# pairlab/leibnizgym

Measured on AMD Instinct MI355X. Metric: env-steps/sec (whole node), trifinger_difficulty_4 @65536 envs, 1/2/4/8 GPUs, higher is better.
Workload: dtype f32

## Files before the change

### leibnizgym_amd/csrc/tf_roles.h

```cpp
#pragma once
#include <type_traits>

#include "tf_contact.h"

#define NT 256

enum { M_ACT_IN = 1, M_RESETS = 2, M_TORQUE = 4, M_SIM = 8, M_POST = 16, M_FINISH = 32, M_ACT_RAND = 64  };
#define M_FUSED_STEP (M_ACT_IN | M_RESETS | M_TORQUE | M_SIM | M_POST | M_FINISH)
#define M_FUSED_STEP_RAND (M_FUSED_STEP | M_ACT_RAND)
#define M_FUSED_RESET (M_RESETS | M_TORQUE | M_SIM | M_POST)

#define L_REC(f) (30 * (f))
#define R_A 0
#define R_DIR 6
#define R_RXD 15
#define R_U 24
#define R_DL 27
#define P_AW 0
#define P_BW 3
#define P_MINV 6
#define P_S1 12
#define P_C1 13
#define P_P2 14
#define P_P3 17
// ... 1754 lines not shown
                    const Yaw ym = {m.base_yaw_cos[fm], m.base_yaw_sin[fm], 0.0f, 0.0f, m.base_height};
                    const float ex[3] = {pm.k.c1, 0.0f, -pm.k.s1};
                    float ey[3], aw[3], bw[3];
                    {
                        float g[3], xg[3], ez[3], ab[3], bb[3];
#pragma unroll
                        for (int i = 0; i < 3; ++i) g[i] = FMA(-jx, ex[i], pm.k.p3[i] - pm.k.p2[i]);
                        cross3(ex, g, xg);
#pragma unroll
                        for (int i = 0; i < 3; ++i) { ey[i] = FMA(jy, g[i], -(jz * xg[i])) * inv_j; ez[i] = FMA(jz, g[i], jy * xg[i]) * inv_j; }
#pragma unroll
                        for (int i = 0; i < 3; ++i) {
                            ab[i] = FMA(sh.a[2], ez[i], FMA(sh.a[1], ey[i], FMA(sh.a[0], ex[i], pm.k.p2[i])));
                            bb[i] = FMA(sh.b[2], ez[i], FMA(sh.b[1], ey[i], FMA(sh.b[0], ex[i], pm.k.p2[i])));
                        }
                        base_to_world(ym, ab, aw);
                        base_to_world(ym, bb, bw);
                    }
                    {
                        const int o = o_;
                        const int fd = (fm + o >= 3) ? fm + o - 3 : fm + o;
                        float Pm[3], Pd[3], sp;
                        {
                            float Ad[3], Bd[3];
#pragma unroll
                            for (int j = 0; j < 3; ++j) { Ad[j] = LD(L_REC(fd) + P_AW + j); Bd[j] = LD(L_REC(fd) + P_BW + j); }
                            seg_seg_s(aw, bw, Ad, Bd, Pm, Pd, sp);
                        }
                        const float dv[3] = {Pd[0] - Pm[0], Pd[1] - Pm[1], Pd[2] - Pm[2]};
                        const float dist2 = dot3(dv, dv);
                        const float inv = f_rsqrt(f_max(dist2, 1e-12f));
                        const float dist = dist2 * inv;
                        const float n[3] = {dv[0] * inv, dv[1] * inv, dv[2] * inv};
                        float nm[3];
                        dir_world_to_base(ym, n, nm);
                        const float u1 = dot3(nm, ex), u2 = dot3(nm, ey);
                        const float rho = FMA(sp, sh.rho[1] - sh.rho[0], sh.rho[0]);
                        const float h1 = FMA(sp, sh.w1[1] - sh.w1[0], sh.w1[0]) - rho, h2 = FMA(sp, sh.w2[1] - sh.w2[0], sh.w2[0]) - rho;
                        const float o1 = FMA(sp, sh.o1[1] - sh.o1[0], sh.o1[0]), o2 = FMA(sp, sh.o2[1] - sh.o2[0], sh.o2[0]);
                        const float ext = FMA(o2, u2, FMA(o1, u1, FMA(h2, f_abs(u2), FMA(h1, f_abs(u1), rho))));
                        const float gap = dist - ext - m.cap_radius;
                        if ((dist2 > 1e-12f) && (gap < m.contact_margin)) {
                            float Jd[3], Wd[3], Jm[3], Wm[3], vd[3], vm[3];
                            {
                                const Yaw yd = {m.base_yaw_cos[fd], m.base_yaw_sin[fd], 0.0f, 0.0f, m.base_height};
                                FingerPubRegs pd;
                                read_pub(lds, lane, fd, pd);
                                float C[3], Cb_[3], L1[3], L2[3], L3[3], nb[3];
#pragma unroll
                                for (int j = 0; j < 3; ++j) C[j] = FMA(-m.cap_radius, n[j], Pd[j]);
                                world_to_base(yd, C, Cb_);
                                levers(pd.k, Cb_, L1, L2, L3);
                                dir_world_to_base(yd, n, nb);
                                Jd[0] = dot3(L1, nb); Jd[1] = dot3(L2, nb); Jd[2] = dot3(L3, nb);
                                sym3_mul(pd.k.Minv, Jd, Wd);
                            }
                            {
                                float C[3], Cb_[3], L1[3], L2[3], L3[3];
#pragma unroll
                                for (int j = 0; j < 3; ++j) C[j] = FMA(ext, n[j], Pm[j]);
                                world_to_base(ym, C, Cb_);
                                levers(pm.k, Cb_, L1, L2, L3);
                                Jm[0] = dot3(L1, nm); Jm[1] = dot3(L2, nm); Jm[2] = 0.0f;
                                sym3_mul(pm.k.Minv, Jm, Wm);
                            }
#pragma unroll
                            for (int j = 0; j < 3; ++j) { vd[j] = LD(L_REC(fd) + P_VQ + j); vm[j] = LD(L_REC(fm) + P_VQ + j); }
                            const float vn0 = dot3(Jd, vd) - dot3(Jm, vm);
                            if (contact_live(m, gap, vn0, h)) {
                                const float bias = contact_bias(m, gap, vn0, inv_h, rest_ff);
                                const float lam = f_max(-(vn0 + bias) * f_rcp2(dot3(Jd, Wd) + dot3(Jm, Wm)), 0.0f);
#pragma unroll
                                for (int j = 0; j < 3; ++j) {
                                    const float dd = Wd[j] * lam, dm = Wm[j] * lam;
                                    if (dd != 0.0f) LD(L_VQFF + 3 * fd + j) = LD(L_VQFF + 3 * fd + j) + dd;
                                    if (dm != 0.0f) LD(L_VQFF + 3 * fm + j) = LD(L_VQFF + 3 * fm + j) - dm;
                                }
                            }
                        }
                    }
                }
            }
            STAMP(sb_ + 2);
            BAR();
            STAMP(sb_ + 3);
            if constexpr (WIDE) {
#include "tf_floor_corners.inc"
            }
            STAMP(sb_ + 4);
            BAR();
            STAMP(sb_ + 5);
            if constexpr (WIDE && !BOXK) {
            Twist tw;
#pragma unroll
            for (int j = 0; j < 3; ++j) { tw.p[j].x = v[j]; tw.p[j].y = w[j]; }
            float2v mI; mI.x = inv_m; mI.y = inv_I;
            float cDinv[9], cbias[3], clam[9], Km[9];
            float2v rec[27];
#pragma unroll
            for (int f = 0; f < 3; ++f) {
                const int rb = L_REC(f);
                cbias[f] = LD(L_INIT + f);
#pragma unroll
                for (int d = 0; d < 3; ++d) { cDinv[3 * f + d] = LD(L_VQFF + 3 * f + d); clam[3 * f + d] = LD(rb + R_DL + d); Km[3 * f + d] = LD(rb + R_A + d); }
#pragma unroll
                for (int j = 0; j < 9; ++j) { rec[9 * f + j].x = LD(rb + R_DIR + j); rec[9 * f + j].y = LD(rb + R_RXD + j); }
                if (cDinv[3 * f] > 0.0f) {
#pragma unroll
                    for (int d = 0; d < 3; ++d) pk_row_apply_neg(&rec[9 * f + 3 * d], clam[3 * f + d], mI, tw);
                }
            }
#pragma unroll
            for (int c = 0; c < 4; ++c) {
                if (fDinv[3 * c] > 0.0f) {
                    cz_apply(&fr_[3 * c], flam[3 * c], mI, tw);
                    cx_apply(&fr_[3 * c], flam[3 * c + 1], mI, tw);
                    cy_apply(&fr_[3 * c], flam[3 * c + 2], mI, tw);
                }
            }
#pragma unroll
            for (int c = 0; c < 4; ++c) {
                const int wb = L_WALL + 12 * c;
                if (c < 2) {
                    if (slot_any[c] && w_D[3 * c] > 0.0f) {
                        wn_apply(&w_n[2 * c], &w_a[3 * c], w_lam[3 * c], mI, tw);
                        wt_apply(&w_n[2 * c], &w_b[3 * c], w_lam[3 * c + 1], mI, tw);
                        cz_apply(&w_r[3 * c], w_lam[3 * c + 2], mI, tw);
                    }
                } else if (slot_any[c] && LD(wb + 5) > 0.0f) {
                    float r[3] = {LD(wb), LD(wb + 1), LD(wb + 2)}, n[2] = {LD(wb + 3), LD(wb + 4)};
                    float a[3], b[3];
                    wall_arm_n(r, n, a);
                    wall_arm_t(r, n, b);
                    wn_apply(n, a, LD(wb + 9), mI, tw);
                    wt_apply(n, b, LD(wb + 10), mI, tw);
                    cz_apply(r, LD(wb + 11), mI, tw);
                }
            }
            if constexpr (SURF) {
                if (__builtin_expect(cone_any != 0u, 0)) {
#pragma unroll 1
                    for (int c = 0; c < 4; ++c) {
                        const int cb = L_CONE + 22 * c, wb = L_WALL + 12 * c;
                        if (((cone_any >> c) & 1u) && LD(cb + 18) > 0.0f) {
#pragma unroll 1
                            for (int d = 0; d < 3; ++d) pk_row_apply_lds(lds, lane, cb + 6 * d, LD(wb + 9 + d), mI, tw);
                        }
                    }
                }
            }
            uint32_t t_wait = 0u, t_fc = 0u, t_floor = 0u;
            STAMP(sb_ + 9);
            for (int it = 0; it < P.iters; ++it) {
                const uint32_t tf0_ = NOW();
                const bool last = it == P.iters - 1;
                float uu[9];
#pragma unroll
                for (int f = 0; f < 3; ++f) {
#pragma unroll
                    for (int j = 0; j < 3; ++j) uu[3 * f + j] = LD(L_REC(f) + R_U + j);
                }
#pragma unroll
                for (int f = 0; f < 3; ++f) {
#ifdef TF_DIAG_NO_FC
                    if (false) {
#else
                    if (cDinv[3 * f] > 0.0f) {
#endif
                        const int rb = L_REC(f);
                        const float2v* R = &rec[9 * f];
                        float vr[3], dl[3];
                        {
                            float2v p0 = R[0] * tw.p[0], p1 = R[3] * tw.p[0], p2 = R[6] * tw.p[0];
                            p0 = pk_fma(R[1], tw.p[1], p0); p1 = pk_fma(R[4], tw.p[1], p1); p2 = pk_fma(R[7], tw.p[1], p2);
                            p0 = pk_fma(R[2], tw.p[2], p0); p1 = pk_fma(R[5], tw.p[2], p1); p2 = pk_fma(R[8], tw.p[2], p2);
                            vr[0] = uu[3 * f] - (p0.x + p0.y); vr[1] = uu[3 * f + 1] - (p1.x + p1.y); vr[2] = uu[3 * f + 2] - (p2.x + p2.y);
                        }
                        dl[0] = solve_normal(clam[3 * f], cDinv[3 * f], vr[0], cbias[f]);
                        vr[1] = FMA(Km[3 * f], dl[0], vr[1]);
                        dl[1] = solve_tangent(clam[3 * f + 1], cDinv[3 * f + 1], vr[1], mu_fc * clam[3 * f]);
                        vr[2] = FMA(Km[3 * f + 2], dl[1], FMA(Km[3 * f + 1], dl[0], vr[2]));
                        dl[2] = solve_tangent(clam[3 * f + 2], cDinv[3 * f + 2], vr[2], mu_fc * clam[3 * f]);
#pragma unroll
                        for (int d = 0; d < 3; ++d) {
                            LD(rb + R_DL + d) = dl[d];
                            pk_row_apply_neg(&R[3 * d], dl[d], mI, tw);
                        }
                    }
                }
                t_fc += NOW() - tf0_;
                { const uint32_t t0_ = NOW(); BAR(); t_wait += NOW() - t0_; }
#pragma unroll
                for (int c = 0; c < 4; ++c) {
                    const float* r = &fr_[3 * c];
#ifdef TF_DIAG_NO_FLOOR
                    if (false) {
#else
                    if (fDinv[3 * c] > 0.0f) {
#endif
                        float dl = solve_normal(flam[3 * c], fDinv[3 * c], cz_vrel(r, tw), fbias[c]);
                        cz_apply(r, dl, mI, tw);
                        dl = solve_tangent(flam[3 * c + 1], fDinv[3 * c + 1], cx_vrel(r, tw), mu_cf * flam[3 * c]);
                        cx_apply(r, dl, mI, tw);
                        dl = solve_tangent(flam[3 * c + 2], fDinv[3 * c + 2], cy_vrel(r, tw), mu_cf * flam[3 * c]);
                        cy_apply(r, dl, mI, tw);
                    }
                }
                t_floor += NOW() - tf0_;
#pragma unroll
                for (int c = 0; c < 4; ++c) {
#ifdef TF_DIAG_NO_WALL
                    continue;
#endif
                    if (!slot_any[c]) continue;
                    const int wb = L_WALL + 12 * c;
                    if (c < 2) {
                        float dl = solve_normal(w_lam[3 * c], w_D[3 * c], wn_vrel(&w_n[2 * c], &w_a[3 * c], tw), w_bias[c]);
                        wn_apply(&w_n[2 * c], &w_a[3 * c], dl, mI, tw);
                        dl = solve_tangent(w_lam[3 * c + 1], w_D[3 * c + 1], wt_vrel(&w_n[2 * c], &w_b[3 * c], tw), mu_cw * w_lam[3 * c]);
                        wt_apply(&w_n[2 * c], &w_b[3 * c], dl, mI, tw);
                        dl = solve_tangent(w_lam[3 * c + 2], w_D[3 * c + 2], cz_vrel(&w_r[3 * c], tw), mu_cw * w_lam[3 * c]);
                        cz_apply(&w_r[3 * c], dl, mI, tw);
                        if (last && w_D[3 * c] > 0.0f) {
#pragma unroll
                            for (int d = 0; d < 3; ++d) LD(wb + 9 + d) = w_lam[3 * c + d];
                        }
                    } else {
                        float r[3] = {LD(wb), LD(wb + 1), LD(wb + 2)}, n[2] = {LD(wb + 3), LD(wb + 4)};
                        float Dinv[3] = {LD(wb + 5), LD(wb + 6), LD(wb + 7)}, bias = LD(wb + 8);
                        float lam[3] = {LD(wb + 9), LD(wb + 10), LD(wb + 11)};
                        float a[3], b[3];
                        wall_arm_n(r, n, a);
                        wall_arm_t(r, n, b);
                        float dl = solve_normal(lam[0], Dinv[0], wn_vrel(n, a, tw), bias);
                        wn_apply(n, a, dl, mI, tw);
                        dl = solve_tangent(lam[1], Dinv[1], wt_vrel(n, b, tw), mu_cw * lam[0]);
                        wt_apply(n, b, dl, mI, tw);
                        dl = solve_tangent(lam[2], Dinv[2], cz_vrel(r, tw), mu_cw * lam[0]);
                        cz_apply(r, dl, mI, tw);
                        if (Dinv[0] > 0.0f) {
#pragma unroll
                            for (int d = 0; d < 3; ++d) LD(wb + 9 + d) = lam[d];
                        }
                    }
                }
                if constexpr (SURF) {
                    if (__builtin_expect(cone_any != 0u, 0)) {
#pragma unroll
                    for (int c = 0; c < 4; ++c) {
                        const int cb = L_CONE + 22 * c, wb = L_WALL + 12 * c;
                        if (((cone_any >> c) & 1u) && LD(cb + 18) > 0.0f) {
                            float lim = 0.0f;
#pragma unroll
                            for (int d = 0; d < 3; ++d) {
                                const float vr = pk_row_vel_lds(lds, lane, cb + 6 * d, tw);
                                float lam = LD(wb + 9 + d);
                                const float dl = (d == 0) ? solve_normal(lam, LD(cb + 18), vr, LD(cb + 21)) : solve_tangent(lam, LD(cb + 18 + d), vr, lim);
                                lim = (d == 0) ? mu_cw * lam : lim;
                                LD(wb + 9 + d) = lam;
                                pk_row_apply_lds(lds, lane, cb + 6 * d, dl, mI, tw);
                            }
                        }
                    }
                    }
                }
                if (last) {
#pragma unroll
                    for (int f = 0; f < 3; ++f) {
                        const int rb = L_REC(f);
                        float ftv[3] = {0.0f, 0.0f, 0.0f}, Fc[3] = {0.0f, 0.0f, 0.0f};
                        if (cDinv[3 * f] > 0.0f) {
#pragma unroll
                            for (int j = 0; j < 3; ++j) {
                                ftv[j] = FMA(rec[9 * f + 6 + j].x, clam[3 * f + 2], rec[9 * f + 3 + j].x * clam[3 * f + 1]);
                                Fc[j] = FMA(rec[9 * f + j].x, clam[3 * f], ftv[j]) * inv_h;
                            }
                        }
                        LD(L_INIT + f) = clam[3 * f];
#pragma unroll
                        for (int j = 0; j < 3; ++j) { LD(rb + R_A + j) = ftv[j]; LD(rb + R_A + 3 + j) = Fc[j]; }
                    }
                }
                { const uint32_t t0_ = NOW(); BAR(); t_wait += NOW() - t0_; }
            }
            STAMP(sb_ + 6);
            STAMPV(sb_ + 8, t_wait);
            STAMPV(sb_ + 10, t_fc);
            STAMPV(sb_ + 11, t_floor);
#pragma unroll
            for (int j = 0; j < 3; ++j) { v[j] = tw.p[j].x; w[j] = tw.p[j].y; }
            } else {
            float cDinv[9], cbias[3], clam[9];
            constexpr int NRR = WIDE ? 27 : 1, NRA = WIDE ? 9 : 1;
            float rA[NRA], rDir[NRR], rRxd[NRR];
            if (WIDE) {
#pragma unroll
                for (int f = 0; f < 3; ++f) {
#pragma unroll
                    for (int j = 0; j < 3; ++j) rA[(3 * f + j) % NRA] = LD(L_REC(f) + R_A + j);
#pragma unroll
                    for (int j = 0; j < 9; ++j) { rDir[(9 * f + j) % NRR] = LD(L_REC(f) + R_DIR + j); rRxd[(9 * f + j) % NRR] = LD(L_REC(f) + R_RXD + j); }
                }
            }
#pragma unroll
            for (int f = 0; f < 3; ++f) {
                const int rb = L_REC(f);
                cbias[f] = LD(L_INIT + f);
#pragma unroll
                for (int d = 0; d < 3; ++d) { cDinv[3 * f + d] = LD(L_VQFF + 3 * f + d); clam[3 * f + d] = LD(rb + R_DL + d); }
                if (cDinv[3 * f] > 0.0f) {
#pragma unroll
                    for (int d = 0; d < 3; ++d) {
                        float dir[3], rxd[3];
#pragma unroll
                        for (int j = 0; j < 3; ++j) { dir[j] = WIDE ? rDir[(9 * f + 3 * d + j) % NRR] : LD(rb + R_DIR + 3 * d + j); rxd[j] = WIDE ? rRxd[(9 * f + 3 * d + j) % NRR] : LD(rb + R_RXD + 3 * d + j); }
                        float sc = clam[3 * f + d] * inv_m, qq = clam[3 * f + d] * inv_I;
#pragma unroll
                        for (int j = 0; j < 3; ++j) { v[j] = FMA(-dir[j], sc, v[j]); w[j] = FMA(-rxd[j], qq, w[j]); }
                    }
                }
            }
#pragma unroll
            for (int c = 0; c < 4; ++c) {
                if (fDinv[3 * c] > 0.0f) {
                    if (__builtin_expect(box, 0)) {
                        float S[6];
#pragma unroll
                        for (int e = 0; e < 6; ++e) S[e] = LD(L_POSE_S + e);
#pragma unroll
                        for (int d = 0; d < 3; ++d) {
                            float n[3], a[3];
                            box_axis(d, n);
                            box_arm(S, &fr_[3 * c], n, a);
                            g_apply(n, a, flam[3 * c + d], inv_m, inv_I, v, w);
                        }
                    } else {
                        cz_apply(&fr_[3 * c], flam[3 * c], inv_m, inv_I, v, w);
                        cx_apply(&fr_[3 * c], flam[3 * c + 1], inv_m, inv_I, v, w);
                        cy_apply(&fr_[3 * c], flam[3 * c + 2], inv_m, inv_I, v, w);
                    }
                }
            }
            {
#pragma unroll
            for (int c = 0; c < 4; ++c) {
                const int wb = L_WALL + 12 * c;
                if (WREG && c < 2) {
                    if (slot_any[c] && w_D[3 * c] > 0.0f) {
                        wn_apply(&w_n[2 * c], &w_a[3 * c], w_lam[3 * c], inv_m, inv_I, v, w);
                        wt_apply(&w_n[2 * c], &w_b[3 * c], w_lam[3 * c + 1], inv_m, inv_I, v, w);
                        cz_apply(&w_r[3 * c], w_lam[3 * c + 2], inv_m, inv_I, v, w);
                    }
                } else
                if (slot_any[c] && LD(wb + 5) > 0.0f) {
                    float r[3] = {LD(wb), LD(wb + 1), LD(wb + 2)}, n[2] = {LD(wb + 3), LD(wb + 4)};
                    float a[3], b[3], c3[3];
                    wall_arms(box, lds, lane, r, n, a, b, c3);
                    wn_apply(n, a, LD(wb + 9), inv_m, inv_I, v, w);
                    wt_apply(n, b, LD(wb + 10), inv_m, inv_I, v, w);
                    if (__builtin_expect(box, 0)) { float ez[3]; box_axis(0, ez); g_apply(ez, c3, LD(wb + 11), inv_m, inv_I, v, w); }
                    else cz_apply(r, LD(wb + 11), inv_m, inv_I, v, w);
                }
            }
            }
            uint32_t t_wait = 0u, t_fc = 0u, t_floor = 0u;
            STAMP(sb_ + 9);
            for (int it = 0; it < P.iters; ++it) {
                const uint32_t tf0_ = NOW();
                const bool last = it == P.iters - 1;
                float uu[9];
                if (WIDE) {
#pragma unroll
                    for (int f = 0; f < 3; ++f) {
#pragma unroll
                        for (int j = 0; j < 3; ++j) uu[3 * f + j] = LD(L_REC(f) + R_U + j);
                    }
                }
#pragma unroll
                for (int f = 0; f < 3; ++f) {
                    const int rb = L_REC(f);
                    if (cDinv[3 * f] > 0.0f) {
                        float Km[3], u[3], dirs[9], rxds[9], vr[3], dl[3];
#pragma unroll
                        for (int j = 0; j < 3; ++j) { Km[j] = WIDE ? rA[(3 * f + j) % NRA] : LD(rb + R_A + j); u[j] = WIDE ? uu[3 * f + j] : LD(rb + R_U + j); }
#pragma unroll
                        for (int j = 0; j < 9; ++j) { dirs[j] = WIDE ? rDir[(9 * f + j) % NRR] : LD(rb + R_DIR + j); rxds[j] = WIDE ? rRxd[(9 * f + j) % NRR] : LD(rb + R_RXD + j); }
#pragma unroll
                        for (int d = 0; d < 3; ++d) vr[d] = u[d] - (dot3(&dirs[3 * d], v) + dot3(&rxds[3 * d], w));
                        dl[0] = solve_normal(clam[3 * f], cDinv[3 * f], vr[0], cbias[f]);
                        vr[1] = FMA(Km[0], dl[0], vr[1]);
                        dl[1] = solve_tangent(clam[3 * f + 1], cDinv[3 * f + 1], vr[1], mu_fc * clam[3 * f]);
                        vr[2] = FMA(Km[2], dl[1], FMA(Km[1], dl[0], vr[2]));
                        dl[2] = solve_tangent(clam[3 * f + 2], cDinv[3 * f + 2], vr[2], mu_fc * clam[3 * f]);
#pragma unroll
                        for (int d = 0; d < 3; ++d) {
                            LD(rb + R_DL + d) = dl[d];
                            const float sc = dl[d] * inv_m, qq = dl[d] * inv_I;
#pragma unroll
                            for (int j = 0; j < 3; ++j) { v[j] = FMA(-dirs[3 * d + j], sc, v[j]); w[j] = FMA(-rxds[3 * d + j], qq, w[j]); }
                        }
                    }
                }
                t_fc += NOW() - tf0_;
                { const uint32_t t0_ = NOW(); BAR(); t_wait += NOW() - t0_; }
#pragma unroll
                for (int c = 0; c < 4; ++c) {
                    const float* r = &fr_[3 * c];
                    if (__builtin_expect(box, 0)) {
                        if (fDinv[3 * c] > 0.0f) {
                            float S[6];
#pragma unroll
                            for (int e = 0; e < 6; ++e) S[e] = LD(L_POSE_S + e);
#pragma unroll
                            for (int d = 0; d < 3; ++d) {
                                float n[3], a[3];
                                box_axis(d, n);
                                box_arm(S, r, n, a);
                                const float vrel = g_vrel(n, a, v, w);
                                const float dlb = (d == 0) ? solve_normal(flam[3 * c], fDinv[3 * c], vrel, fbias[c])
                                                           : solve_tangent(flam[3 * c + d], fDinv[3 * c + d], vrel, mu_cf * flam[3 * c]);
                                g_apply(n, a, dlb, inv_m, inv_I, v, w);
                            }
                        }
                    } else
                    if (fDinv[3 * c] > 0.0f) {
                        float dl = solve_normal(flam[3 * c], fDinv[3 * c], cz_vrel(r, v, w), fbias[c]);
                        cz_apply(r, dl, inv_m, inv_I, v, w);
                        dl = solve_tangent(flam[3 * c + 1], fDinv[3 * c + 1], cx_vrel(r, v, w), mu_cf * flam[3 * c]);
                        cx_apply(r, dl, inv_m, inv_I, v, w);
                        dl = solve_tangent(flam[3 * c + 2], fDinv[3 * c + 2], cy_vrel(r, v, w), mu_cf * flam[3 * c]);
                        cy_apply(r, dl, inv_m, inv_I, v, w);
                    }
                }
                t_floor += NOW() - tf0_;
                {
#pragma unroll
                for (int c = 0; c < 4; ++c) {
                    if (!slot_any[c]) continue;
                    const int wb = L_WALL + 12 * c;
                    if (WREG && c < 2) {
                        float dl = solve_normal(w_lam[3 * c], w_D[3 * c], wn_vrel(&w_n[2 * c], &w_a[3 * c], v, w), w_bias[c]);
                        wn_apply(&w_n[2 * c], &w_a[3 * c], dl, inv_m, inv_I, v, w);
                        dl = solve_tangent(w_lam[3 * c + 1], w_D[3 * c + 1], wt_vrel(&w_n[2 * c], &w_b[3 * c], v, w), mu_cw * w_lam[3 * c]);
                        wt_apply(&w_n[2 * c], &w_b[3 * c], dl, inv_m, inv_I, v, w);
                        dl = solve_tangent(w_lam[3 * c + 2], w_D[3 * c + 2], cz_vrel(&w_r[3 * c], v, w), mu_cw * w_lam[3 * c]);
                        cz_apply(&w_r[3 * c], dl, inv_m, inv_I, v, w);
                        if (last && w_D[3 * c] > 0.0f) {
#pragma unroll
                            for (int d = 0; d < 3; ++d) LD(wb + 9 + d) = w_lam[3 * c + d];
                        }
                    } else {
                        float r[3] = {LD(wb), LD(wb + 1), LD(wb + 2)}, n[2] = {LD(wb + 3), LD(wb + 4)};
                        float Dinv[3] = {LD(wb + 5), LD(wb + 6), LD(wb + 7)}, bias = LD(wb + 8);
                        float lam[3] = {LD(wb + 9), LD(wb + 10), LD(wb + 11)};
                        float a[3], b[3], c3[3];
                        wall_arms(box, lds, lane, r, n, a, b, c3);
                        float dl = solve_normal(lam[0], Dinv[0], wn_vrel(n, a, v, w), bias);
                        wn_apply(n, a, dl, inv_m, inv_I, v, w);
                        dl = solve_tangent(lam[1], Dinv[1], wt_vrel(n, b, v, w), mu_cw * lam[0]);
                        wt_apply(n, b, dl, inv_m, inv_I, v, w);
                        if (__builtin_expect(box, 0)) {
                            float ez[3];
                            box_axis(0, ez);
                            dl = solve_tangent(lam[2], Dinv[2], g_vrel(ez, c3, v, w), mu_cw * lam[0]);
                            g_apply(ez, c3, dl, inv_m, inv_I, v, w);
                        } else {
                            dl = solve_tangent(lam[2], Dinv[2], cz_vrel(r, v, w), mu_cw * lam[0]);
                            cz_apply(r, dl, inv_m, inv_I, v, w);
                        }
                        if (Dinv[0] > 0.0f) {
#pragma unroll
                            for (int d = 0; d < 3; ++d) LD(wb + 9 + d) = lam[d];
                        }
                    }
                }
                }
                if (last) {
#pragma unroll
                    for (int f = 0; f < 3; ++f) {
                        const int rb = L_REC(f);
                        float ftv[3] = {0.0f, 0.0f, 0.0f}, Fc[3] = {0.0f, 0.0f, 0.0f};
                        if (cDinv[3 * f] > 0.0f) {
                            float dirs[9];
#pragma unroll
                            for (int j = 0; j < 9; ++j) dirs[j] = WIDE ? rDir[(9 * f + j) % NRR] : LD(rb + R_DIR + j);
#pragma unroll
                            for (int j = 0; j < 3; ++j) {
                                ftv[j] = FMA(dirs[6 + j], clam[3 * f + 2], dirs[3 + j] * clam[3 * f + 1]);
                                Fc[j] = FMA(dirs[j], clam[3 * f], ftv[j]) * inv_h;
                            }
                        }
                        LD(L_INIT + f) = clam[3 * f];
#pragma unroll
                        for (int j = 0; j < 3; ++j) { LD(rb + R_A + j) = ftv[j]; LD(rb + R_A + 3 + j) = Fc[j]; }
                    }
                }
                { const uint32_t t0_ = NOW(); BAR(); t_wait += NOW() - t0_; }
            }
            STAMP(sb_ + 6);
            STAMPV(sb_ + 8, t_wait);
            STAMPV(sb_ + 10, t_fc);
            STAMPV(sb_ + 11, t_floor);
            }
#pragma unroll
            for (int j = 0; j < 12; ++j) lam_cf[j] = flam[j];
            if (__builtin_expect(box, 0)) {
                float S[6], ww[3];
#pragma unroll
                for (int e = 0; e < 6; ++e) S[e] = LD(L_POSE_S + e);
                sym3_mul(S, w, ww);
#pragma unroll
                for (int j = 0; j < 3; ++j) w[j] = ww[j];
            }
#pragma unroll
            for (int j = 0; j < 3; ++j) {
                cv[j] = v[j]; cw[j] = w[j];
                cp[j] = FMA(h, v[j], cp[j]);
            }
            quat_integrate(cq, cw, h);
            STAMP(sb_ + 7);
        }
#pragma unroll
        for (int c = 0; c < 4; ++c) {
#pragma unroll
            for (int d = 0; d < 3; ++d) lam_cw[3 * c + d] = LD(L_WALL + 12 * c + 9 + d);
        }
        __builtin_amdgcn_s_setprio(0);
    }
    STAMP(30);
    StatsTicket tk;
    tk.mine = 0ull; tk.old = 0ull;
    if (MODE & (M_POST | M_FINISH)) {
        c_reset = P.reset_buf[(unsigned)cx.i] != 0;
        c_goal_reset = P.goal_reset_buf[(unsigned)cx.i] != 0;
        c_successes = P.successes[(unsigned)cx.i] != 0;
        c_steps = (int)P.steps[(unsigned)cx.i];
    }
    if (MODE & M_POST) {
        float gp[3], gq[4], prev_obj[7];
#pragma unroll
        for (int j = 0; j < 3; ++j) gp[j] = LDST(TF_S_GOAL_P + j);
#pragma unroll
        for (int j = 0; j < 4; ++j) gq[j] = LDST(TF_S_GOAL_Q + j);
#pragma unroll
        for (int j = 0; j < 7; ++j) prev_obj[j] = LDST(TF_S_PREV_OBJ_P + j);
        LaneStats st;
        stats_zero(st);
        st.resets = n_resets;
        {
            float acc = 0.0f;
#pragma unroll
            for (int j = 0; j < 3; ++j) acc = acc + cp[j] * 0.0f + cv[j] * 0.0f + cw[j] * 0.0f;
#pragma unroll
            for (int j = 0; j < 4; ++j) acc = acc + cq[j] * 0.0f;
            LD(L_NAN + 3) = (acc == 0.0f) ? 0.0f : 1.0f;
        }
        float o_dist = 0.0f, o_ang = 0.0f, o_r[4] = {0.0f, 0.0f, 0.0f, 0.0f};
        auto object_terms = [&]() __attribute__((always_inline)) {
            const RewardCoef& rc = sa.rc;
            o_dist = norm3d(cp, gp);
            o_r[0] = rc.c_dist * lgsk(o_dist, 50.0f);
            o_ang = quat_diff_rad(cq, gq);
            o_r[1] = rc.w_rot * (rc.rot_num / (rc.rot_scale * f_abs(o_ang) + rc.rot_scale));
            const float ang_prev = quat_diff_rad(&prev_obj[3], gq);
            o_r[2] = rc.w_rot_delta * (rc.rot_delta_sched * (f_abs(o_ang) - f_abs(ang_prev)));
            o_r[3] = rc.w_move * (o_dist - norm3d(prev_obj, gp));
        };
        if (!IS_RESET) {
            object_terms();
            if (!WIDE) { LD(L_OTERM) = o_dist; LD(L_OTERM + 1) = o_ang; LD(L_OTERM + 2) = o_r[0]; LD(L_OTERM + 3) = o_r[1]; LD(L_OTERM + 4) = o_r[2]; LD(L_OTERM + 5) = o_r[3]; }
        }
        STAMP(31);
        BAR();
        STAMP(32);
        const bool guarded = (LD(L_NAN) + LD(L_NAN + 1) + LD(L_NAN + 2) + LD(L_NAN + 3)) != 0.0f;
        if (__builtin_expect(guarded, 0)) {
            cp[0] = 0.0f; cp[1] = 0.0f; cp[2] = m.obj_min_height;
            cq[0] = 0.0f; cq[1] = 0.0f; cq[2] = 0.0f; cq[3] = 1.0f;
#pragma unroll
            for (int k = 0; k < 3; ++k) { cv[k] = 0.0f; cw[k] = 0.0f; }
            if (cx.valid) P.reset_buf[(unsigned)cx.i] = 1;
            c_reset = true;
            st.nonfinite += cx.valid ? 1.0f : 0.0f;
            if (!IS_RESET) {
                object_terms();
                if (!WIDE) { LD(L_OTERM) = o_dist; LD(L_OTERM + 1) = o_ang; LD(L_OTERM + 2) = o_r[0]; LD(L_OTERM + 3) = o_r[1]; LD(L_OTERM + 4) = o_r[2]; LD(L_OTERM + 5) = o_r[3]; }
            }
        }
        const float co = P.clip_obs;
        const bool nrm = P.normalize_obs != 0;
        float* row = &lds[lane * TW];
#pragma unroll
        for (int j = 0; j < 3; ++j) { row[18 + j] = emit_scaled(cp[j], PLO(j), 0.3f, nrm, co); row[25 + j] = emit_scaled(gp[j], PLO(j), 0.3f, nrm, co); }
#pragma unroll
        for (int j = 0; j < 4; ++j) { row[21 + j] = emit_scaled(cq[j], -1.0f, 1.0f, nrm, co); row[28 + j] = emit_scaled(gq[j], -1.0f, 1.0f, nrm, co); }
        if (ASYM) {
#pragma unroll
            for (int j = 0; j < 3; ++j) { row[OD + j] = emit_scaled(cv[j], -0.5f, 0.5f, nrm, co); row[OD + 3 + j] = emit_scaled(cw[j], -0.5f, 0.5f, nrm, co); }
        }
        auto add_noise = [&]() {
            float nz[28];
#pragma unroll
            for (int b = 4; b < 7; ++b) rng4(P, gid, sa.frame, RNG_OBS_NOISE + (uint32_t)b, &nz[4 * b]);
#pragma unroll
            for (int jj = 18; jj < 25; ++jj) row[jj] = f_clamp(FMA(P.dr_obs_noise, 2.0f * nz[jj] - 1.0f, row[jj]), -co, co);
        };
        if (DR && !ASYM && P.dr_obs_noise > 0.0f) add_noise();
        STAMP(33);
        BAR();
        STAMP(34);
        if (!IS_RESET) {
            float tips[9], tip_prev[9];
#pragma unroll
            for (int f = 0; f < 3; ++f) {
#pragma unroll
                for (int j = 0; j < 3; ++j) { tips[3 * f + j] = LD(L_XCH + 6 * f + j); tip_prev[3 * f + j] = LD(L_XCH + 6 * f + 3 + j); }
            }
            const RewardCoef& rc = sa.rc;
            float r[6];
            {
                float s = 0.0f;
                s = s + (norm_p3(&tips[0], cp, P.norm_p) - norm_p3(&tip_prev[0], prev_obj, P.norm_p));
                s = s + (norm_p3(&tips[3], cp, P.norm_p) - norm_p3(&tip_prev[3], prev_obj, P.norm_p));
                s = s + (norm_p3(&tips[6], cp, P.norm_p) - norm_p3(&tip_prev[6], prev_obj, P.norm_p));
                r[0] = rc.c_reach * s;
            }
            {
                float s = 0.0f;
#pragma unroll
                for (int j = 0; j < 9; ++j) s = s + LD(L_VSQ + j);
                r[1] = rc.c_move_pen * s;
            }
            if (!WIDE) { o_dist = LD(L_OTERM); o_ang = LD(L_OTERM + 1); o_r[0] = LD(L_OTERM + 2); o_r[1] = LD(L_OTERM + 3); o_r[2] = LD(L_OTERM + 4); o_r[3] = LD(L_OTERM + 5); }
            const float dist = o_dist, ang = o_ang;
            r[2] = o_r[0]; r[3] = o_r[1]; r[4] = o_r[2]; r[5] = o_r[3];
            float total = 0.0f;
#pragma unroll
            for (int t = 0; t < 6; ++t) {
                r[t] = guarded ? 0.0f : r[t];
                if (P.rew_active[t]) { total = total + r[t]; st.rew[t] += cx.valid ? r[t] : 0.0f; }
            }
            bool pos_ok = dist <= P.pos_tol;
            bool ori_ok = ang <= P.ori_tol;
            st.pos_cnt += (cx.valid && pos_ok) ? 1.0f : 0.0f;
            st.ori_cnt += (cx.valid && ori_ok) ? 1.0f : 0.0f;
            bool done;
            if (P.task_difficulty < 4) done = pos_ok;
            else if (P.task_difficulty == 4) done = pos_ok && ori_ok;
            else done = ori_ok;
            bool succ = c_successes;
            if (P.success_activate) {
                if (done) total = total + P.success_bonus;
                if (cx.valid) P.goal_reset_buf[(unsigned)cx.i] = (uint8_t)done;
                c_goal_reset = done;
                succ = succ || done;
            } else {
                succ = c_goal_reset && succ;
            }
            c_successes = succ;
            if (cx.valid) {
                P.successes[(unsigned)cx.i] = (uint8_t)succ;
                P.reward[(unsigned)cx.i] = total;
            }
            st.succ += (cx.valid && succ) ? 1.0f : 0.0f;
        }
        STAMP(36);
        stats_begin(P, st, lane, tk);
        STAMP(37);
        if (DR && ASYM && P.dr_obs_noise > 0.0f) {
            BAR();
            add_noise();
            BAR();
        }
    }
    if (MODE & (M_RESETS | M_SIM | M_POST)) {
#pragma unroll
        for (int j = 0; j < 3; ++j) { STST(TF_S_CUBE_P + j, cp[j]); STST(TF_S_CUBE_V + j, cv[j]); STST(TF_S_CUBE_W + j, cw[j]); }
#pragma unroll
        for (int j = 0; j < 4; ++j) STST(TF_S_CUBE_Q + j, cq[j]);
    }
    if (MODE & (M_RESETS | M_SIM)) {
#pragma unroll
        for (int j = 0; j < 12; ++j) STST(TF_S_LAM_CF + j, lam_cf[j]);
        STST(TF_S_CF_FACE, cf_face); STST(TF_S_CW_FACE, cw_face);
        if (__builtin_expect(cw_face != 0.0f, 0)) {
#pragma unroll
            for (int j = 0; j < 12; ++j) STST(TF_S_LAM_CW + j, lam_cw[j]);
        }
    }
    if ((MODE & M_POST) && P.goal_rotation_activate) {
        float gq2[4], gw2[3];
#pragma unroll
        for (int j = 0; j < 4; ++j) gq2[j] = LDST(TF_S_GOAL_Q + j);
#pragma unroll
        for (int j = 0; j < 3; ++j) gw2[j] = LDST(TF_S_GOAL_W + j);
        const int nadv = ((MODE & M_SIM) ? sa.nsim : P.control_decimation) * P.substeps;
        for (int s = 0; s < nadv; ++s) quat_integrate(gq2, gw2, P.hsub);
#pragma unroll
        for (int j = 0; j < 4; ++j) STST(TF_S_GOAL_Q + j, gq2[j]);
    }
    STAMP(38);
    if (MODE & M_FINISH) {
        if (cx.valid) {
            int sN = c_steps + 1;
            P.steps[(unsigned)cx.i] = (int64_t)sN;
            bool rb = c_reset;
            if (P.episode_length > 0 && sN >= P.episode_length) { rb = true; P.reset_buf[(unsigned)cx.i] = 1; }
            P.dones[(unsigned)cx.i] = (uint8_t)(rb && c_goal_reset);
        }
    }
    STAMP(39);
    if (MODE & M_POST) stats_end(P, lane, tk);
    STAMP(35);
    STAMPV(40, __builtin_amdgcn_s_getreg((31 << 11) | 4));
    STAMPV(41, __builtin_amdgcn_s_getreg((31 << 11) | 20));
}
```

Baseline: 1.003 billion.

## Compact active fingertip contacts via per-lane LDS indices in narrow solver path

```diff
diff --git a/leibnizgym_amd/csrc/tf_roles.h b/leibnizgym_amd/csrc/tf_roles.h
--- a/leibnizgym_amd/csrc/tf_roles.h
+++ b/leibnizgym_amd/csrc/tf_roles.h
@@ -2080,21 +2080,63 @@
                     for (int j = 0; j < 9; ++j) { rDir[(9 * f + j) % NRR] = LD(L_REC(f) + R_DIR + j); rRxd[(9 * f + j) % NRR] = LD(L_REC(f) + R_RXD + j); }
                 }
             }
-#pragma unroll
-            for (int f = 0; f < 3; ++f) {
-                const int rb = L_REC(f);
-                cbias[f] = LD(L_INIT + f);
-#pragma unroll
-                for (int d = 0; d < 3; ++d) { cDinv[3 * f + d] = LD(L_VQFF + 3 * f + d); clam[3 * f + d] = LD(rb + R_DL + d); }
-                if (cDinv[3 * f] > 0.0f) {
-#pragma unroll
-                    for (int d = 0; d < 3; ++d) {
-                        float dir[3], rxd[3];
-#pragma unroll
-                        for (int j = 0; j < 3; ++j) { dir[j] = WIDE ? rDir[(9 * f + 3 * d + j) % NRR] : LD(rb + R_DIR + 3 * d + j); rxd[j] = WIDE ? rRxd[(9 * f + 3 * d + j) % NRR] : LD(rb + R_RXD + 3 * d + j); }
-                        float sc = clam[3 * f + d] * inv_m, qq = clam[3 * f + d] * inv_I;
-#pragma unroll
-                        for (int j = 0; j < 3; ++j) { v[j] = FMA(-dir[j], sc, v[j]); w[j] = FMA(-rxd[j], qq, w[j]); }
+            int fc_ix[3] = {L_REC(2) * WAVE + lane, L_REC(2) * WAVE + lane, L_REC(2) * WAVE + lane};
+#define FC_REC(k, slot) lds[fc_ix[k] + (slot) * WAVE]
+            if constexpr (!WIDE) {
+                float sD[9], sb[3], sl[9];
+#pragma unroll
+                for (int f = 0; f < 3; ++f) {
+                    sb[f] = LD(L_INIT + f);
+#pragma unroll
+                    for (int d = 0; d < 3; ++d) { sD[3 * f + d] = LD(L_VQFF + 3 * f + d); sl[3 * f + d] = LD(L_REC(f) + R_DL + d); }
+                }
+#pragma unroll 1
+                for (int f = 0; f < 3; ++f) {
+                    const int rb = L_REC(f);
+                    if ((f == 0 ? sD[0] : (f == 1 ? sD[3] : sD[6])) > 0.0f) {
+#pragma unroll
+                        for (int d = 0; d < 3; ++d) {
+                            float dir[3], rxd[3];
+#pragma unroll
+                            for (int j = 0; j < 3; ++j) { dir[j] = LD(rb + R_DIR + 3 * d + j); rxd[j] = LD(rb + R_RXD + 3 * d + j); }
+                            const float l = f == 0 ? sl[d] : (f == 1 ? sl[3 + d] : sl[6 + d]);
+                            float sc = l * inv_m, qq = l * inv_I;
+#pragma unroll
+                            for (int j = 0; j < 3; ++j) { v[j] = FMA(-dir[j], sc, v[j]); w[j] = FMA(-rxd[j], qq, w[j]); }
+                        }
+                    }
+                }
+                const bool l0 = sD[0] > 0.0f, l1 = sD[3] > 0.0f, l01 = l0 && l1;
+                fc_ix[0] = (l0 ? L_REC(0) : (l1 ? L_REC(1) : L_REC(2))) * WAVE + lane;
+                fc_ix[1] = (l01 ? L_REC(1) : L_REC(2)) * WAVE + lane;
+                cbias[0] = l0 ? sb[0] : (l1 ? sb[1] : sb[2]); cbias[1] = l01 ? sb[1] : sb[2]; cbias[2] = sb[2];
+#pragma unroll
+                for (int d = 0; d < 3; ++d) {
+                    cDinv[d] = l0 ? sD[d] : (l1 ? sD[3 + d] : sD[6 + d]); cDinv[3 + d] = l01 ? sD[3 + d] : sD[6 + d]; cDinv[6 + d] = sD[6 + d];
+                    clam[d] = l0 ? sl[d] : (l1 ? sl[3 + d] : sl[6 + d]); clam[3 + d] = l01 ? sl[3 + d] : sl[6 + d]; clam[6 + d] = sl[6 + d];
+                }
+                cDinv[3] = (l0 || l1) ? cDinv[3] : 0.0f;
+                cDinv[6] = l01 ? sD[6] : 0.0f;
+                if (cDinv[6] > 0.0f) {
+#pragma unroll
+                    for (int d = 0; d < 3; ++d) LD(L_REC(2) + R_A + 3 + d) = clam[6 + d];
+                }
+            } else {
+#pragma unroll
+                for (int f = 0; f < 3; ++f) {
+                    const int rb = L_REC(f);
+                    cbias[f] = LD(L_INIT + f);
+#pragma unroll
+                    for (int d = 0; d < 3; ++d) { cDinv[3 * f + d] = LD(L_VQFF + 3 * f + d); clam[3 * f + d] = LD(rb + R_DL + d); }
+                    if (cDinv[3 * f] > 0.0f) {
+#pragma unroll
+                        for (int d = 0; d < 3; ++d) {
+                            const float* dir = &rDir[(9 * f + 3 * d) % NRR];
+                            const float* rxd = &rRxd[(9 * f + 3 * d) % NRR];
+                            float sc = clam[3 * f + d] * inv_m, qq = clam[3 * f + d] * inv_I;
+#pragma unroll
+                            for (int j = 0; j < 3; ++j) { v[j] = FMA(-dir[j], sc, v[j]); w[j] = FMA(-rxd[j], qq, w[j]); }
+                        }
                     }
                 }
             }
@@ -2160,11 +2202,16 @@
                     if (cDinv[3 * f] > 0.0f) {
                         float Km[3], u[3], dirs[9], rxds[9], vr[3], dl[3];
 #pragma unroll
-                        for (int j = 0; j < 3; ++j) { Km[j] = WIDE ? rA[(3 * f + j) % NRA] : LD(rb + R_A + j); u[j] = WIDE ? uu[3 * f + j] : LD(rb + R_U + j); }
-#pragma unroll
-                        for (int j = 0; j < 9; ++j) { dirs[j] = WIDE ? rDir[(9 * f + j) % NRR] : LD(rb + R_DIR + j); rxds[j] = WIDE ? rRxd[(9 * f + j) % NRR] : LD(rb + R_RXD + j); }
+                        for (int j = 0; j < 3; ++j) { Km[j] = WIDE ? rA[(3 * f + j) % NRA] : FC_REC(f, R_A + j); u[j] = WIDE ? uu[3 * f + j] : FC_REC(f, R_U + j); }
+#pragma unroll
+                        for (int j = 0; j < 9; ++j) { dirs[j] = WIDE ? rDir[(9 * f + j) % NRR] : FC_REC(f, R_DIR + j); rxds[j] = WIDE ? rRxd[(9 * f + j) % NRR] : FC_REC(f, R_RXD + j); }
 #pragma unroll
                         for (int d = 0; d < 3; ++d) vr[d] = u[d] - (dot3(&dirs[3 * d], v) + dot3(&rxds[3 * d], w));
+                        if (!WIDE && f == 2) {
+                            cbias[2] = LD(L_INIT + 2);
+#pragma unroll
+                            for (int d = 0; d < 3; ++d) clam[6 + d] = LD(L_REC(2) + R_A + 3 + d);
+                        }
                         dl[0] = solve_normal(clam[3 * f], cDinv[3 * f], vr[0], cbias[f]);
                         vr[1] = FMA(Km[0], dl[0], vr[1]);
                         dl[1] = solve_tangent(clam[3 * f + 1], cDinv[3 * f + 1], vr[1], mu_fc * clam[3 * f]);
@@ -2172,7 +2219,8 @@
                         dl[2] = solve_tangent(clam[3 * f + 2], cDinv[3 * f + 2], vr[2], mu_fc * clam[3 * f]);
 #pragma unroll
                         for (int d = 0; d < 3; ++d) {
-                            LD(rb + R_DL + d) = dl[d];
+                            if constexpr (WIDE) LD(rb + R_DL + d) = dl[d]; else FC_REC(f, R_DL + d) = dl[d];
+                            if (!WIDE && f == 2) LD(L_REC(2) + R_A + 3 + d) = clam[6 + d];
                             const float sc = dl[d] * inv_m, qq = dl[d] * inv_I;
 #pragma unroll
                             for (int j = 0; j < 3; ++j) { v[j] = FMA(-dirs[3 * d + j], sc, v[j]); w[j] = FMA(-rxds[3 * d + j], qq, w[j]); }
@@ -2253,15 +2301,45 @@
                     }
                 }
                 }
+                if (!WIDE && last) {
+#pragma unroll
+                    for (int k = 0; k < 2; ++k) {
+                        if (cDinv[3 * k] > 0.0f) {
+#pragma unroll
+                            for (int d = 0; d < 3; ++d) FC_REC(k, R_A + 3 + d) = clam[3 * k + d];
+                        }
+                    }
+#pragma unroll
+                    for (int f = 0; f < 3; ++f) {
+                        const int rb = L_REC(f);
+                        float ftv[3] = {0.0f, 0.0f, 0.0f}, Fc[3] = {0.0f, 0.0f, 0.0f};
+                        float l0 = LD(rb + R_DL);
+                        if (LD(L_VQFF + 3 * f) > 0.0f) {
+                            float dirs[9], l[3];
+#pragma unroll
+                            for (int j = 0; j < 9; ++j) dirs[j] = LD(rb + R_DIR + j);
+#pragma unroll
+                            for (int d = 0; d < 3; ++d) l[d] = LD(rb + R_A + 3 + d);
+#pragma unroll
+                            for (int j = 0; j < 3; ++j) {
+                                ftv[j] = FMA(dirs[6 + j], l[2], dirs[3 + j] * l[1]);
+                                Fc[j] = FMA(dirs[j], l[0], ftv[j]) * inv_h;
+                            }
+                            l0 = l[0];
+                        }
+                        LD(L_INIT + f) = l0;
+#pragma unroll
+                        for (int j = 0; j < 3; ++j) { LD(rb + R_A + j) = ftv[j]; LD(rb + R_A + 3 + j) = Fc[j]; }
+                    }
+                }
+                if constexpr (WIDE) {
                 if (last) {
 #pragma unroll
                     for (int f = 0; f < 3; ++f) {
                         const int rb = L_REC(f);
                         float ftv[3] = {0.0f, 0.0f, 0.0f}, Fc[3] = {0.0f, 0.0f, 0.0f};
                         if (cDinv[3 * f] > 0.0f) {
-                            float dirs[9];
-#pragma unroll
-                            for (int j = 0; j < 9; ++j) dirs[j] = WIDE ? rDir[(9 * f + j) % NRR] : LD(rb + R_DIR + j);
+                            const float* dirs = &rDir[(9 * f) % NRR];
 #pragma unroll
                             for (int j = 0; j < 3; ++j) {
                                 ftv[j] = FMA(dirs[6 + j], clam[3 * f + 2], dirs[3 + j] * clam[3 * f + 1]);
@@ -2273,12 +2351,14 @@
                         for (int j = 0; j < 3; ++j) { LD(rb + R_A + j) = ftv[j]; LD(rb + R_A + 3 + j) = Fc[j]; }
                     }
                 }
+                }
                 { const uint32_t t0_ = NOW(); BAR(); t_wait += NOW() - t0_; }
             }
             STAMP(sb_ + 6);
             STAMPV(sb_ + 8, t_wait);
             STAMPV(sb_ + 10, t_fc);
             STAMPV(sb_ + 11, t_floor);
+#undef FC_REC
             }
 #pragma unroll
             for (int j = 0; j < 12; ++j) lam_cf[j] = flam[j];
```

Result: faster. 1.018 billion, median of 6 (+1.4%).
